# LANL-Seismoacoustics/GeoAc

Measured on AMD Instinct MI355X. Metric: RK4 ray-steps/sec, GeoAcGlobal 360x90 ToyAtmo fan; arrivals within 1e-6 of ref, higher is better.
Workload: dtype f64; 1 GPU; GeoAcGlobal -prop ToyAtmo.met, 360 az x 90 incl = 32400 rays (phi step 1 deg), bounces=2, CalcAmp=True, WriteRays=False, rng_max=1500; rays_per_gpu=32400, ray_steps_per_pass=874273730, parallelism=azimuth-sharded x1

## Files before the change

geoac_amd/csrc/geoac_api.cpp:

```cpp
#include <hip/hip_runtime.h>
#include <math.h>
#include <cmath>
#include <stdio.h>
#include <stdlib.h>
#include <string.h>
#include <ctype.h>
#include <errno.h>
#include <algorithm>
#include <atomic>
#include <memory>
#include <mutex>
#include <string>
#include <thread>
#include <vector>

#include "../../include/geoac_hip.h"
#include "../../include/geoac_probe.h"
#include "../../include/geoac_host.h"
#include "geoac_device.h"
#include "geoac_map_int.h"
#include "geoac_stations_int.h"
#include "geoac_tubemap_int.h"
#include "geoac_refine_int.h"

// ... 120 lines not shown
    hipStream_t pp_stream = nullptr;
    hipStream_t acc_stream = nullptr;
    std::vector<hipEvent_t> evp;
    hipStream_t rk4b_stream = nullptr;
    std::vector<hipEvent_t> evj;
    DevBuf ev_row[3], ev_m[3], ev_amp[3], nev[3], smp_out;
    long long smp_cap = 4ll << 20;
    unsigned long long n_samples = 0;
    unsigned long long* h_counters = nullptr;
    int n_rays = 0, n_pad = 0, legs = 0;
    double ms_total = 0, ms_rk4 = 0, ms_post = 0;
    unsigned long long n_epochs = 0, path_bytes_w = 0, path_bytes_r = 0, total_steps = 0, err_flags = 0;
    int s_rows_override = 0;
    bool no_overlap = false;
    int pp_blocks = 0;
    double pair_frac = -1.0;
    double stagger_frac = -1.0;
    double stagger_rows = -1.0;
    double hybrid_rows = -1.0;
    bool two_chunks = false;
    bool trace_epochs = false;
    bool no_gate = false;
    bool no_pair = false;
    bool grid_build_host = false;
    int ev_slack = 72;
    int trio = 0;
    int duo = 0;
    bool abs_table = true;
    DevBuf atab;
    std::vector<double> atab_mkey;
    DevBuf ppfix;
    double atab_tol = 1e-10;
    int ppfix_cap = 1 << 20;
    unsigned long long atmo_version = 0, atab_version = ~0ull;
    double atab_key[7] = {0, 0, 0, 0, 0, 0, 0};
    int atab_entries = 0, atab_flagged = 0;
    double atab_worst = 0;
    unsigned long long pp_fixup_segments = 0;
    int n_members = 1;
    int mem_slots = 0;
    std::vector<double> ens_T, ens_rho, ens_sl;
    std::vector<double> mconsts;
    DevBuf d_mconsts;
    int n_src = 1;
    std::vector<double> sources;
    int layout_members = 1;
// ... 64 lines not shown
const char* geoac_last_error(geoac_ctx* ctx){ return ctx ? ctx->err.c_str() : ""; }

int geoac_default_params(int eqset, geoac_params* p){
    if(!p) return GEOAC_E_INVALID;
    memset(p, 0, sizeof(*p));
    p->ds_min = 0.001; p->ds_max = 0.5;
    if(eqset == GEOAC_EQ_GLOBAL || eqset == GEOAC_EQ_GLOBAL_RNGDEP){
        p->ray_limit = 10000.0;
        p->range_limit = 1500.0;
        p->r_earth = 6370.0;
        p->src[0] = 0.0; p->src[1] = 30.0; p->src[2] = 0.0;
    } else {
        p->ray_limit = 5000.0;
        p->range_limit = 10000.0;
        p->r_earth = 0.0;
    }
    p->vert_limit = NAN;
    p->z_grnd = 0.0; p->tweak_abs = 0.3; p->freq = 0.1;
    p->bounces = 2; p->calc_amp = 1; p->mode = 0; p->sample_stride = 25;
    for(int q = 0; q < 4; q++) p->xy_limits[q] = NAN;
    return GEOAC_OK;
}

static const char* const kOptionNames[] = {
    "S_ROWS", "NO_OVERLAP", "PP_BLOCKS", "ABS_TABLE", "ABS_TABLE_TOL", "PPFIX_CAP", "DUO", "TRIO", "EV_SLACK", "NO_PAIR", "PAIR_FRAC", "HYBRID_ROWS", "STAGGER_FRAC", "STAGGER_ROWS", "TWO_CHUNKS", "TRACE_EPOCHS", "NO_GATE", "SORT", "TILE", "PP_ONETRIP", "PP_LDS_TABLE", "PP_LDS_PAD", "CU_SPLIT", "CHUNK_GIB", "ACCUM_BATCH",
    "NO_QUAD", "GRID_LANES", "OCT", "HEX", "SPREAD", "COMPACT", "QUAD_CACHE", "GRID_COOP", "SUB_EPOCHS", "SUB_MIN_WAVES", "SUB_TEST_STALL", "SMP_CAP", "GRID_BUILD", nullptr };
const char* const* geoac_option_names(void){ return kOptionNames; }

int geoac_set_option(geoac_ctx* ctx, const char* key, const char* value){
    if(!ctx || !key || !value) return GEOAC_E_INVALID;
    std::string k(key);
    if(k.rfind("GEOAC_", 0) == 0) k = k.substr(6);
    for(char& c : k) c = (char)toupper((unsigned char)c);
    bool int_ok = false, dbl_ok = false;
    long long lv = 0; double dv = 0.0;
    { char* end = nullptr; errno = 0; lv = strtoll(value, &end, 10); int_ok = (end != value && *end == 0 && errno == 0); }
    { char* end = nullptr; errno = 0; dv = strtod(value, &end); dbl_ok = (end != value && *end == 0 && errno == 0 && dv == dv); }
    const int iv = (int)lv;
    auto bad = [&](const char* want){ return fail(ctx, GEOAC_E_INVALID, "set_option: " + k + "=" + value + ": expected " + want); };
    auto flag = [&](bool& dst) -> int { if(!int_ok || (lv != 0 && lv != 1)) return bad("0 or 1"); dst = lv != 0; return GEOAC_OK; };
    if(k == "S_ROWS"){ if(!int_ok || lv < 0 || lv > 0x7fffffff) return bad("a row count >= 0 (0: sized from the free memory)"); ctx->s_rows_override = iv; }
    else if(k == "NO_OVERLAP") return flag(ctx->no_overlap);
    else if(k == "PP_BLOCKS"){ if(!int_ok || lv < 0 || lv > 0x7fffffff) return bad("a block count >= 0"); ctx->pp_blocks = iv; }
    else if(k == "ABS_TABLE") return flag(ctx->abs_table);
    else if(k == "ABS_TABLE_TOL"){ if(!dbl_ok || !(dv > 0.0)) return bad("a tolerance > 0"); ctx->atab_tol = dv; }
    else if(k == "PPFIX_CAP"){ if(!int_ok || lv <= 0 || lv > 0x3fffffff) return bad("a capacity > 0"); ctx->ppfix_cap = iv; }
    else if(k == "DUO"){
        if(!int_ok || lv < 0 || lv > 3) return bad("0..3");
        if(lv && !geoac_build_has_ab()) return fail(ctx, GEOAC_E_UNSUPPORTED, "set_option: DUO: the wave-specialised kernel is part of A/B builds only (make AB=1)");
        ctx->duo = iv;
    }
    else if(k == "TRIO"){
        if(!int_ok || lv < 0 || lv > 31) return bad("0, 1 (3, 5, 11, 27: timing diagnostics)");
        if(lv && !geoac_build_has_ab()) return fail(ctx, GEOAC_E_UNSUPPORTED, "set_option: TRIO: the three-wave kernel is part of A/B builds only (make AB=1)");
        ctx->trio = iv;
    }
    else if(k == "EV_SLACK"){ if(!int_ok || lv < 0 || lv > 1000000) return bad("a slot count >= 0"); ctx->ev_slack = iv; }
    else if(k == "NO_PAIR") return flag(ctx->no_pair);
    else if(k == "PAIR_FRAC"){ if(!dbl_ok || dv < 0.0 || dv > 1.0) return bad("a share in [0, 1]"); ctx->pair_frac = dv; }
    else if(k == "STAGGER_FRAC"){ if(!dbl_ok || dv < -1.0 || dv > 0.9) return bad("a share in [0, 0.9] (0: off), or -1 (by launch plan)"); ctx->stagger_frac = dv; }
    else if(k == "STAGGER_ROWS"){ if(!dbl_ok || !(dv > 0.0 && dv <= 1.0)) return bad("a ratio in (0, 1]"); ctx->stagger_rows = dv; }
    else if(k == "HYBRID_ROWS"){ if(!dbl_ok || !(dv > 0.0 && dv <= 1.0)) return bad("a ratio in (0, 1]"); ctx->hybrid_rows = dv; }
    else if(k == "TWO_CHUNKS") return flag(ctx->two_chunks);
    else if(k == "TRACE_EPOCHS") return flag(ctx->trace_epochs);
    else if(k == "NO_GATE") return flag(ctx->no_gate);
    else if(k == "SORT") return flag(ctx->sort_rays);
    else if(k == "TILE") return flag(ctx->tile_rays);
    else if(k == "PP_ONETRIP"){ if(!int_ok || lv < -1 || lv > 1) return bad("0, 1 or -1 (by launch plan)"); ctx->pp_onetrip = iv; }
    else if(k == "CHUNK_GIB"){ if(!int_ok || lv < 1 || lv > 256) return bad("GiB per path chunk in 1 .. 256"); ctx->chunk_gib = iv; }
    else if(k == "ACCUM_BATCH"){ if(!int_ok || lv < -1 || lv > 1) return bad("0, 1 or -1 (by launch plan: the late epochs)"); ctx->accum_batch = iv; }
    else if(k == "CU_SPLIT"){ if(!int_ok || lv < -1 || lv > 248) return bad("compute units for the post-pass, 0 .. 248 (0: no partition), or -1 (by launch plan)"); ctx->cu_split = iv; }
    else if(k == "PP_LDS_PAD"){ if(!int_ok || lv < -1 || lv > 160 * 1024) return bad("bytes of LDS in 0 .. 163840, or -1 (by launch plan)"); ctx->pp_lds_pad = iv; }
    else if(k == "PP_LDS_TABLE"){ if(!int_ok || lv < -1 || lv > 1) return bad("0, 1 or -1 (by launch plan)"); ctx->pp_lds_table = iv; }
    else if(k == "NO_QUAD") return flag(ctx->no_quad);
    else if(k == "GRID_LANES"){
        if(!int_ok || !(iv == 0 || iv == 1 || iv == 2 || iv == 4 || iv == 8 || iv == 16)) return bad("0, 1, 2, 4, 8 or 16");
        if(iv == 2 && !geoac_build_has_ab()) return fail(ctx, GEOAC_E_UNSUPPORTED, "set_option: GRID_LANES=2: the grid sets' two-lane kernels are part of A/B builds only (make AB=1)");
        ctx->grid_lanes = iv;
    }
    else if(k == "OCT") return flag(ctx->oct);
    else if(k == "HEX") return flag(ctx->hex);
    else if(k == "SPREAD"){ if(!int_ok || lv < 0 || lv > 64 || (lv & (lv - 1))) return bad("0 (by launch plan) or a power of two up to 64"); ctx->spread_override = iv; }
    else if(k == "COMPACT") return flag(ctx->compact);
    else if(k == "QUAD_CACHE") return flag(ctx->quad_cache);
    else if(k == "GRID_COOP") return flag(ctx->grid_coop);
    else if(k == "SUB_EPOCHS"){ if(!int_ok || lv < 1 || lv > 16) return bad("1..16"); ctx->sub_epochs = iv; }
// ... 472 lines not shown
    const bool is_global = (ctx->eqset == GEOAC_EQ_GLOBAL);
    const bool is_sph = is_global || ctx->eqset == GEOAC_EQ_GLOBAL_RNGDEP;
    if(is_global){ P.E = p.calc_amp ? 18 : 6; P.pathw = 6; }
    else if(ctx->eqset == GEOAC_EQ_3D){ P.E = p.calc_amp ? 12 : 4; P.pathw = 4; }
    else if(is_grid){ P.E = p.calc_amp ? 18 : 6; P.pathw = 6; }
    else { P.E = p.calc_amp ? 6 : 3; P.pathw = 2; }
    P.rays_form = ((p.mode & (GEOAC_MODE_WRITE_RAYS | GEOAC_MODE_WRITE_CAUSTICS)) != 0 || ctx->eqset == GEOAC_EQ_2D) ? 1 : 0;
    P.nseg = ctx->n_nodes - 1;
    P.step_limit = (long long)(p.ray_limit * (int)(1.0 / (p.ds_min * 10)));
    if(P.step_limit > 0x7fffffffLL) P.step_limit = 0x7fffffffLL;
    if(P.step_limit < 2) P.step_limit = 2;
    P.x_min = ctx->x[0]; P.x_max = ctx->x[ctx->n_nodes - 1];
    P.ds_min = p.ds_min; P.ds_max = p.ds_max;
    P.r_earth = is_sph ? p.r_earth : 0.0; P.z_grnd = p.z_grnd;
    P.ground = P.r_earth + p.z_grnd;
    P.vert_limit = p.vert_limit; P.range_limit = p.range_limit;
    if(p.range_limit >= 0.0){ const double l2 = p.range_limit * p.range_limit; P.range_sq[0] = l2 * (1.0 - 1e-12); P.range_sq[1] = l2 * (1.0 + 1e-12); }
    else { P.range_sq[0] = 0.0; P.range_sq[1] = -1.0; }
    if(is_global){
        double half = p.range_limit / (2.0 * p.r_earth);
        if(half >= kPi / 2.0){ P.range_thresh = 2.0; P.range_skip = 1e300; }
        else if(half <= 0.0){ P.range_thresh = -1.0; P.range_skip = -1.0; }
        else { double s = sin(half); P.range_thresh = s * s; P.range_skip = half * (1.0 - 1e-9); }
    }
    P.src[0] = p.src[0]; P.src[1] = p.src[1]; P.src[2] = p.src[2];
    P.freq = p.freq; P.tweak_abs = p.tweak_abs;
    {
        P.sb_const[0] = pow(10.0, -0.67887); P.sb_const[1] = pow(10.0, -0.10744); P.sb_const[2] = pow(10, -3.3979);
        P.sb_const[3] = 5.0 / sqrt(21.0); P.sb_const[4] = sqrt(3.0 / 7.0);
        P.src_trig[0] = sin(p.src[1] * kPi / 180.0); P.src_trig[1] = cos(p.src[1] * kPi / 180.0);
        if(is_grid){ P.T_o = P.P_o = 0.0; P.c000 = 0.0; } else {
        const size_t nn = (size_t)ctx->n_nodes;
        ctx->mconsts.assign((size_t)K * GEOAC_MEMP, 0.0);
        std::vector<double> Tm, rm;
        for(int m = 0; m < K; m++){
        const bool prof = K > 1;
        if(prof){ Tm.assign(ctx->ens_T.begin() + m * nn, ctx->ens_T.begin() + (m + 1) * nn); rm.assign(ctx->ens_rho.begin() + m * nn, ctx->ens_rho.begin() + (m + 1) * nn); }
        const std::vector<double>& Tv = prof ? Tm : ctx->T;
        const std::vector<double>& rv = prof ? rm : ctx->rho;
        const double* slm = prof ? ctx->ens_sl.data() + 4 * nn * m : ctx->sl.data();
        double Tg = host_spline_f(ctx->x, Tv, slm, p.z_grnd);
        double rg = host_spline_f(ctx->x, rv, slm + 3 * nn, p.z_grnd);
        double cg = sqrt(kGamR * Tg) * 1000.0;
        P.T_o = cg * cg / (kRgas * kGam);
        P.cbrt_To = cbrt(P.T_o);
        P.P_o = rg * (cg * cg) / kGam * 1000.0;
// ... 744 lines not shown
```

geoac_amd/csrc/geoac_device.h:

```cpp
#ifndef GEOAC_DEVICE_H_
#define GEOAC_DEVICE_H_

#include <stdint.h>

#define GEOAC_SEGW      14
#define GEOAC_MAXE      18
#define GEOAC_MAXLEGS   64
#define GEOAC_ATABW     20
#define GEOAC_LAT_OFF   1024
#define GEOAC_LAT_N     2049
#define GEOAC_PP_ROWS   16
#define GEOAC_CNT_PPFLAG 28

enum {
    ST_Y0     = 0,
    ST_K      = 18,
    ST_LEG    = 19,
    ST_DONE   = 20,
    ST_HMAX   = 21,
    ST_C0     = 22,
    ST_NU0    = 23,
    ST_AUX0   = 24,
    ST_SEG    = 30,
    ST_TT     = 31,
    ST_AT     = 32,
    ST_PLEG   = 33,
    ST_LTT    = 34,
    ST_LAT    = 35,
    ST_YM2    = 36,
    ST_DPREV  = 54,
    ST_NSTATE = 55
};

struct GeoacDevParams {
// ... 2 lines not shown
    int     E, pathw;
    int     nseg;
    int     s_rows;
    int     table_in_lds;
    int     live_slot;
    int     slot_lo, slot_hi;
    int     lanes_per_ray;
    int     duo;
    int     trio;
    int     spread;
    int     quad_cache;
    int     coop;
    int     seg_safe;
    int     pp_blocks;
    int     rays_form;
    long long step_limit;
    double  x_min, x_max;
    double  ds_min, ds_max;
    double  ground;
    double  r_earth, z_grnd;
    double  vert_limit, range_limit, range_thresh;
    double  range_sq[2];
    double  range_skip;
    double  src[3];
    double  freq, tweak_abs;
    double  T_o, P_o;
    double  cbrt_To;
    double  c000;
    double  src_trig[2];
    double  sb_const[5];
    const double* seg;
    const double* rho;
    int*    ppfix;
    int     ppfix_cap;
    int     pp_lds_pad;
    int     accum_batch;
    int     pp_lds_table;
    int     pp_onetrip;
    const double* atab;
    const double* lat_trig;
    int           atab_on;
    double        atab_D;
    double        atab_lo;
    double        seg_per_x;
    int           gnx, gny;
    double        g_lo[2], g_hi[2];
// ... 55 lines not shown
```

geoac_amd/csrc/geoac_kernels.hip:

```cpp
#include <hip/hip_runtime.h>
#include <math.h>
#include <type_traits>
#include "geoac_device.h"
#include "../../include/geoac_hip.h"

#define DEVINL __device__ __forceinline__
#ifndef GEOAC_CACHE_REG_STATE
#define GEOAC_CACHE_REG_STATE 0
#endif
#ifndef GEOAC_OCT_LDS_STATE
#define GEOAC_OCT_LDS_STATE 0
#endif
#define GEOAC_ROT_MAX 1.0e-3

#pragma clang fp contract(off)

#ifndef GEOAC_RCPC
#define GEOAC_RCPC 1
#endif
#ifndef GEOAC_RCPC_EMAX
#define GEOAC_RCPC_EMAX 1.0e-5
#endif
#ifndef GEOAC_AB
#define GEOAC_AB 0
#endif

static constexpr double kPi   = 3.141592653589793238462643;
static constexpr double kGam  = 1.4;
static constexpr double kRgas = 287.05;
static constexpr double kGamR = 0.00040187;

DEVINL double frcp(double x){
    double r = __builtin_amdgcn_rcp(x);
    double e = __builtin_fma(-x, r, 1.0);
    double t = __builtin_fma(e, e, e);
    return __builtin_fma(r, t, r);
}
DEVINL double frsq(double x){
    double y = __builtin_amdgcn_rsq(x);
    double g = x * y;
    double e = __builtin_fma(-g, y, 1.0);
    double p = __builtin_fma(e, 0.375, 0.5);
    return __builtin_fma(y * e, p, y);
}
// ... 185 lines not shown
    double t = x - s[0];
    return __builtin_fma(t, __builtin_fma(t, __builtin_fma(t, q[3], q[2]), q[1]), q[0]);
}

DEVINL void member_view(GeoacDevParams& P, int m){
    const int k = m % P.n_profiles;
    P.seg += (size_t)k * P.nseg * GEOAC_SEGW;
    P.rho += (size_t)k * P.nseg * 4;
    if(P.atab) P.atab += (size_t)k * (P.nseg + 2) * GEOAC_ATABW;
    const double* c = P.mem_consts + (size_t)m * GEOAC_MEMC;
    P.T_o = c[0]; P.P_o = c[1]; P.cbrt_To = c[2]; P.c000 = c[3];
    P.src[0] = c[4]; P.src[1] = c[5]; P.src[2] = c[6];
    P.src_trig[0] = c[7]; P.src_trig[1] = c[8];
}
DEVINL int member_of_slot(const GeoacDevParams& P, int slot){
    const int m = __builtin_amdgcn_readfirstlane(slot) / P.mem_slots;
    return m < P.n_members ? m : P.n_members - 1;
}

struct GlobalStage { double n0, n1, n2, inm, cn, icg, dc, du, dv, v, cg2, ir, ico, sth, cth, H0, K2; };
#define GEOAC_GSTAGE_W 17

struct NoHook { DEVINL void operator()() const {} };
template <bool AMP, int W, typename TabPtr, class HOOK = NoHook, bool ROT0 = false, bool LOCATED = false>
DEVINL void global_base(TabPtr tab, const GeoacDevParams& P, int& seg, double* rec, const double* y, double sth0, double cth0, double dlat, double* dy, GlobalStage& S, const HOOK& hook = HOOK(), double* rcp0 = nullptr, bool first = false){
    const double r = y[0];
    const double n0 = y[3], n1 = y[4], n2 = y[5];
    const double xe = clampq(r, P.x_min, P.x_max);
    double sth, cth;
    if(ROT0){ sth = sth0; cth = cth0; }
    else rot_small(sth0, cth0, dlat, sth, cth);
    const double nn  = __builtin_fma(n0, n0, __builtin_fma(n1, n1, n2 * n2));
    const double inm0 = frsq(nn);
#if GEOAC_RCPC
    double ir, ico;
    if(ROT0 || first){ ir = frcp(r); ico = frcp(cth); rcp0[0] = ir; rcp0[1] = ico; }
    else {
        const double e1 = __builtin_fma(-r, rcp0[0], 1.0), e2 = __builtin_fma(-cth, rcp0[1], 1.0);
        ir = __builtin_fma(rcp0[0], __builtin_fma(e1, e1, e1), rcp0[0]);
        ico = __builtin_fma(rcp0[1], __builtin_fma(e2, e2, e2), rcp0[1]);
        if(__builtin_expect(!(fabs(e2) <= GEOAC_RCPC_EMAX), 0)) ico = frcp(cth);
    }
#else
    const double ir  = frcp(r);
    const double ico = frcp(cth);
#endif
    Atm9 a;
    if(LOCATED) seg_eval_at(rec, xe, a); else seg_cached_eval<W>(tab, P, xe, seg, rec, a);
    hook();
    const double inm = inm0, numag = nn * inm;
    const double u = a.u, v = a.v, du = a.du, dv = a.dv;

    const double qT  = kGamR * a.T;
    const double ic  = frsq(qT);
    const double c   = qT * ic;
    const double hc  = (0.5 * kGamR) * ic;
    const double dc  = hc * a.dT;
    const double cn  = c * inm;
    const double cg0 = cn * n0;
    const double cg1 = __builtin_fma(cn, n1, v);
    const double cg2 = __builtin_fma(cn, n2, u);
    const double icg = frsq(__builtin_fma(cg0, cg0, __builtin_fma(cg1, cg1, cg2 * cg2)));
    const double tn  = sth * ico;
    const double u0 = cg0 * icg, u1 = cg1 * icg, u2 = cg2 * icg;
// ... 52 lines not shown
    const double dcg2 = __builtin_fma(R0, du, a2);
    const double e   = icg * __builtin_fma(D.u0, dcg0, __builtin_fma(D.u1, dcg1, D.u2 * dcg2));
    const double w0 = __builtin_fma(icg, dcg0, -D.u0 * e);
    const double w1 = __builtin_fma(icg, dcg1, -D.u1 * e);
    const double w2 = __builtin_fma(icg, dcg2, -D.u2 * e);
    const double dG1 = -R0 * D.ir2;
    const double dG2 = D.G2 * __builtin_fma(D.tn, R1, -R0 * ir);
    const double s22 = __builtin_fma(m2, cg2, n2 * dcg2);
    const double dT0 = __builtin_fma(dG1, D.nc12, ir * __builtin_fma(m1, D.cg1, __builtin_fma(n1, dcg1, s22)));
    const double dT1 = __builtin_fma(-D.cnn1, m0, __builtin_fma(-n0, a1, __builtin_fma(D.tn, s22, (D.n2cg2 * R1) * D.ico2)));
    const double dncs = __builtin_fma(m0, cth, __builtin_fma(m1, sth, R1 * __builtin_fma(n1, cth, -n0 * sth)));
    const double dT2 = -__builtin_fma(__builtin_fma(m2, v, n2 * dva), sth,
                         __builtin_fma((n2 * v) * R1, cth, __builtin_fma(a2, D.ncs, D.cnn2 * dncs)));

    dya[0] = w0;
    dya[1] = __builtin_fma(dG1, D.u1, G1 * w1);
    dya[2] = __builtin_fma(dG2, D.u2, D.G2 * w2);
    dya[3] = icg * (__builtin_fma(e, H0, -dT0)
                    - __builtin_fma(dnu, dc, __builtin_fma(m1, dv, __builtin_fma(m2, du, R0 * K2))));
    dya[4] = -icg * __builtin_fma(dG1, D.T1, G1 * dT1);
    dya[5] = -icg * __builtin_fma(dG2, D.T2, D.G2 * dT2);
}

template <bool AMP, int NQ, bool ROT0 = false, typename TabPtr>
DEVINL void global_rhs(TabPtr tab, const GeoacDevParams& P, int& seg, double* rec, const double* y, double sth0, double cth0, double dlat, double* dy, double* rcp0 = nullptr){
    GlobalStage S;
    global_base<AMP, GEOAC_SEGW, TabPtr, NoHook, ROT0>(tab, P, seg, rec, y, sth0, cth0, dlat, dy, S, NoHook(), rcp0);
    if(AMP){
        GlobalDerived D;
        global_derive(S, D);
        #pragma unroll
        for(int q = 0; q < NQ; q++) global_aux(S, D, y + 6 + 6 * q, dy + 6 + 6 * q);
    }
}

struct Medium { double c, dc, u, du, v, dv, rho; };
DEVINL Medium medium_at(const GeoacDevParams& P, double x){
    double xe = clampd(x, P.x_min, P.x_max);
    int k = seg_guess(P.seg, P, xe);
    Atm9 a; seg_eval<false>(P.seg, k, xe, a);
    Medium m;
    m.c = sqrt(kGamR * a.T); m.dc = kGamR / (2.0 * m.c) * a.dT;
    m.u = a.u; m.du = a.du; m.v = a.v; m.dv = a.dv;
    m.rho = rho_eval(P, k, xe);
    return m;
}

DEVINL double global_jacobian(const Medium& m, const double* y){
    double r = y[0], th = y[1];
    double nu_mag = sqrt(y[3] * y[3] + y[4] * y[4] + y[5] * y[5]);
// ... 278 lines not shown
        double MS = 1.0 + (nu0[0] * Mach[0] + nu0[1] * Mach[1] + nu0[2] * Mach[2]);
        y[0] = r0; y[1] = lat0; y[2] = lon0;
        for(int e = 0; e < 3; e++) y[3 + e] = nu0[e] / MS;
        if(AMP){
            double dlt = mlt[0] * Mach[0] + mlt[1] * Mach[1] + mlt[2] * Mach[2];
            double dlp = mlp[0] * Mach[0] + mlp[1] * Mach[1] + mlp[2] * Mach[2];
            for(int e = 0; e < 3; e++){
                y[9 + e]  = mlt[e] / MS - nu0[e] / (MS * MS) * dlt;
                y[15 + e] = mlp[e] / MS - nu0[e] / (MS * MS) * dlp;
            }
        }
        C.c0 = c0; C.nu0 = 1.0 / MS;
        C.a[0] = lat0; fsincos(lat0, C.a[1], C.a[2]);
        C.a[3] = 0.0; C.a[4] = 0.0; C.a[5] = 1.0;
        resume(P, C, y);
    }
    static DEVINL void fan_init(const GeoacDevParams& P){}
    static DEVINL double height(const GeoacDevParams& P, const double* y){ return y[0] - P.r_earth; }
    static DEVINL double above_ground(const GeoacDevParams& P, const double* y){ return y[0] - P.ground; }

    static DEVINL void resume(const GeoacDevParams& P, RayCtx& C, const double* y){
        rot_small(C.a[1], C.a[2], y[1] - C.a[0], C.cur[0], C.cur[1]);
    }
    template <typename TabPtr>
    static DEVINL void rhs(TabPtr tab, const GeoacDevParams& P, int& seg, const RayCtx& C, const double* y0, const double* yt, int stage, double* dy){
        if(stage == 0) global_rhs<AMP, 2, true>(tab, P, seg, C.rec, yt, C.cur[0], C.cur[1], 0.0, dy, C.rcp0);
        else global_rhs<AMP, 2>(tab, P, seg, C.rec, yt, C.cur[0], C.cur[1], yt[1] - y0[1], dy, C.rcp0);
    }
    static DEVINL void checks(const GeoacDevParams& P, RayCtx& C, const double* y, const double* yn, int k, bool& brk, bool& gnd){
        const double lon0 = P.src[2] * kPi / 180.0;
        const double dl = yn[1] - C.a[0], pl = yn[2] - lon0;
        if(__builtin_expect(fabs(dl) > GEOAC_ROT_MAX, 0)){ C.a[0] = yn[1]; fsincos(yn[1], C.a[1], C.a[2]); C.t[0] = C.a[1]; C.t[1] = C.a[2]; }
        else rot_small(C.a[1], C.a[2], dl, C.t[0], C.t[1]);
        bool far = false;
        if(fabs(yn[1] - P.src[1] * kPi / 180.0) * 0.5 + fabs(pl) * 0.5 >= P.range_skip){
            const double dp = pl - C.a[3];
            double tp0, tp1;
            if(__builtin_expect(fabs(dp) > GEOAC_ROT_MAX, 0)){ C.a[3] = pl; fsincos(pl, C.a[4], C.a[5]); tp0 = C.a[4]; tp1 = C.a[5]; }
            else rot_small(C.a[4], C.a[5], dp, tp0, tp1);
            const double sl0 = P.src_trig[0], cl0 = P.src_trig[1];
            double hav = __builtin_fma(cl0 * C.t[1], 0.5 * (1.0 - tp1), 0.5 * (1.0 - __builtin_fma(C.t[1], cl0, C.t[0] * sl0)));
            far = hav > P.range_thresh;
        }
        brk = (yn[0] > P.vert_limit) || far;
        gnd = yn[0] < P.ground;
    }
    static DEVINL void accept(RayCtx& C){ C.cur[0] = C.t[0]; C.cur[1] = C.t[1]; }
    static DEVINL void restart(const GeoacDevParams& P, RayCtx& C, const double* y){
        C.a[0] = y[1]; fsincos(y[1], C.a[1], C.a[2]);
        C.a[3] = y[2] - P.src[2] * kPi / 180.0; fsincos(C.a[3], C.a[4], C.a[5]);
        C.cur[0] = C.a[1]; C.cur[1] = C.a[2];
    }
    static DEVINL void arrival(const GeoacDevParams& P, const RayCtx& C, int slot, const double* yn, double* R){
        const double lat0 = P.src[1] * kPi / 180.0, lon0 = P.src[2] * kPi / 180.0;
        Medium m = medium_at(P, yn[0]);
        double z_src = P.src[0] < P.z_grnd ? P.z_grnd : P.src[0];
        double incl = -asin(m.c / C.c0 * yn[3]) * 180.0 / kPi;
        double baz = 90.0 - atan2(-yn[4], -yn[5]) * 180.0 / kPi;
        if(baz < -180.0) baz += 360.0;
        if(baz > 180.0) baz -= 360.0;
        double g1 = sin((yn[1] - lat0) / 2.0); g1 *= g1;
        double g2 = sin((yn[2] - lon0) / 2.0); g2 = cos(lat0) * cos(yn[1]) * g2 * g2;
        R[GEOAC_REC_INCL] = incl;
        R[GEOAC_REC_BACKAZ] = baz;
        R[GEOAC_REC_RANGE] = 2.0 * P.r_earth * asin(sqrt(g1 + g2));
        if(AMP){
            double amp, D;
            amp_jac(P, C, slot, yn, amp, D);
            R[GEOAC_REC_AMP] = amp;
// ... 52 lines not shown
        G.a0 = an0 + (B[3] - an0) / 2.0; G.a1 = an1 + (B[4] - an1) / 2.0; G.a2 = an2 + (B[5] - an2) / 2.0;
        G.a3 = frsq(G.a0 * G.a0 + G.a1 * G.a1 + G.a2 * G.a2);
        G.x = r;
    }
    static DEVINL double pp_tt(const GeoacDevParams& P, const double* aux, const PPGeom& G, double T, double u, double v){
        double qT = kGamR * T;
        double cn = (qT * frsq(qT)) * G.a3;
        double cp0 = cn * G.a0, cp1 = cn * G.a1 + v, cp2 = cn * G.a2 + u;
        return G.ds_tt * frsq(cp0 * cp0 + cp1 * cp1 + cp2 * cp2);
    }
    static DEVINL void segment(const GeoacDevParams& P, const double* st, size_t np, const double* a, const double* b, double& tt, double& at){
        double A[6], B[6];
        #pragma unroll
        for(int c = 0; c < 6; c++){ A[c] = a[c * np]; B[c] = b[c * np]; }
        pp_exact<EqGlobal<AMP_>>(P, nullptr, A, B, tt, at);
    }
};


struct EqGlobalPair : EqGlobal<true> {
    using Full = EqGlobal<true>;
    static constexpr int E = 12, LANES = 2;
    static constexpr bool SPLIT = true; static constexpr bool ROW_SPLIT = true;
    template <typename TabPtr>
    static DEVINL void rhs(TabPtr tab, const GeoacDevParams& P, int& seg, const RayCtx& C, const double* y0, const double* yt, int stage, double* dy){
        if(stage == 0) global_rhs<true, 1, true>(tab, P, seg, C.rec, yt, C.cur[0], C.cur[1], 0.0, dy, C.rcp0);
        else global_rhs<true, 1>(tab, P, seg, C.rec, yt, C.cur[0], C.cur[1], yt[1] - y0[1], dy, C.rcp0);
    }
    static DEVINL void reflect(const GeoacDevParams& P, const RayCtx& C, const double* yn, double* y, const double* ym2){
        double dr_k = yn[0] - y[0];
        double dr_g = y[0] - P.ground;
        double prev[E];
        #pragma unroll
        for(int e = 0; e < E; e++) prev[e] = y[e] + (y[e] - yn[e]) / dr_k * dr_g;
        Medium mr = medium_at(P, prev[0]);
        double c_ref = mr.c;
        double dnu_r_ds = -1.0 / c_ref * (C.c0 / c_ref * mr.dc + prev[4] * mr.dv + prev[5] * mr.du
                                          + c_ref / prev[0] * (prev[4] * prev[4] + prev[5] * prev[5]));
        #pragma unroll
        for(int e = 0; e < E; e++) y[e] = prev[e];
        y[0] = P.ground;
        y[3] = -prev[3];
        y[6] = -prev[6];
        y[9] = -prev[9] + 2.0 * dnu_r_ds * prev[6] / (c_ref / C.c0 * prev[3]);
    }
};

#pragma clang fp contract(fast)
#include "geoac_rngdep.h"
#ifndef GEOAC_CELL_REGS
// ... 408 lines not shown
        C.a[0] = nu0[0] / M; C.a[1] = nu0[1] / M;
        C.a[2] = mth[0] / M - nu0[0] / (M * M) * dMt;  C.a[3] = mth[1] / M - nu0[1] / (M * M) * dMt;
        C.a[4] = mph[0] / M - nu0[0] / (M * M) * dMp;  C.a[5] = mph[1] / M - nu0[1] / (M * M) * dMp;
        y[0] = P.src[0]; y[1] = P.src[1]; y[2] = z0; y[3] = nu0[2] / M;
        if(AMP){
            y[7]  = mth[2] / M - nu0[2] / (M * M) * dMt;
            y[11] = mph[2] / M - nu0[2] / (M * M) * dMp;
        }
    }
    static DEVINL void fan_init(const GeoacDevParams& P){}
    static DEVINL double height(const GeoacDevParams& P, const double* y){ return y[2]; }
    static DEVINL double above_ground(const GeoacDevParams& P, const double* y){ return y[2] - P.ground; }
    template <typename TabPtr>
    static DEVINL void rhs(TabPtr tab, const GeoacDevParams& P, int& seg, const RayCtx& C, const double* y0, const double* yt, int stage, double* dy){
        cart3_rhs<AMP>(tab, P, seg, C, yt, dy);
    }
    static DEVINL void checks(const GeoacDevParams& P, RayCtx& C, const double* y, const double* yn, int k, bool& brk, bool& gnd){
        const double s2 = yn[0] * yn[0] + yn[1] * yn[1];
        bool far = s2 > P.range_sq[1];
        if(__builtin_expect((s2 >= P.range_sq[0]) & (s2 <= P.range_sq[1]), 0)) far = sqrt(s2) > P.range_limit;
        brk = (yn[2] > P.vert_limit) || far;
        gnd = yn[2] < P.ground;
    }
    static DEVINL void accept(RayCtx& C){}
    static DEVINL void resume(const GeoacDevParams& P, RayCtx& C, const double* y){}
    static DEVINL void restart(const GeoacDevParams& P, RayCtx& C, const double* y){}
    static DEVINL void arrival(const GeoacDevParams& P, const RayCtx& C, int slot, const double* yn, double* R){
        double z0 = P.z_grnd < P.src[2] ? P.src[2] : P.z_grnd;
        Medium mg = medium_at(P, P.z_grnd);
        double incl = -asin(mg.c / C.c0 * yn[3]) * 180.0 / kPi;
        double baz = P.phi_deg[slot] + 180.0;
        while(baz > 180.0) baz -= 360.0;
        while(baz < -180.0) baz += 360.0;
        R[GEOAC_REC_INCL] = incl;
        R[GEOAC_REC_BACKAZ] = baz;
        R[GEOAC_REC_RANGE] = sqrt(yn[0] * yn[0] + yn[1] * yn[1]);
        if(AMP){
            double amp, D;
            amp_jac(P, C, slot, yn, amp, D);
            R[GEOAC_REC_AMP] = amp;
            R[GEOAC_REC_JACOB] = D;
        }
    }
    static DEVINL void amp_jac(const GeoacDevParams& P, const RayCtx& C, int slot, const double* yn, double& amp, double& D){
        double z0 = P.z_grnd < P.src[2] ? P.src[2] : P.z_grnd;
        Medium m = medium_at(P, yn[2]);
// ... 95 lines not shown
    static constexpr bool SPLIT = false;
    static constexpr bool KM2 = true, KM2_MEM = false, HMAX_PER_LEG = false;

    static DEVINL void init(const GeoacDevParams& P, double th, double ph, double* y, RayCtx& C){
        double z0 = P.src[0] < P.z_grnd ? P.z_grnd : P.src[0];
        Medium m = medium_at(P, z0);
        C.a[0] = cos(ph); C.a[1] = sin(ph); C.a[2] = cos(th); C.a[3] = sin(th); C.a[4] = 0.0; C.a[5] = 0.0;
        C.c0 = m.c + m.u * C.a[0] + m.v * C.a[1];
        C.nu0 = 1.0 / C.c0;
        y[0] = 0.0; y[1] = z0; y[2] = C.a[3];
        if(AMP) y[5] = C.a[2];
    }
    static DEVINL void fan_init(const GeoacDevParams& P){}
    static DEVINL double height(const GeoacDevParams& P, const double* y){ return y[1]; }
    static DEVINL double above_ground(const GeoacDevParams& P, const double* y){ return y[1] - P.ground; }
    template <typename TabPtr>
    static DEVINL void rhs(TabPtr tab, const GeoacDevParams& P, int& seg, const RayCtx& C, const double* y0, const double* yt, int stage, double* dy){
        cart2_rhs<AMP>(tab, P, seg, C, yt, dy);
    }
    static DEVINL void checks(const GeoacDevParams& P, RayCtx& C, const double* y, const double* yn, int k, bool& brk, bool& gnd){
        brk = (yn[1] > P.vert_limit) || (yn[0] > P.range_limit);
        gnd = yn[1] < P.ground;
    }
    static DEVINL void accept(RayCtx& C){}
    static DEVINL void resume(const GeoacDevParams& P, RayCtx& C, const double* y){}
    static DEVINL void restart(const GeoacDevParams& P, RayCtx& C, const double* y){}
    static DEVINL void arrival(const GeoacDevParams& P, const RayCtx& C, int slot, const double* yn, double* R){
        R[GEOAC_REC_INCL] = -P.theta_deg[slot];
        R[GEOAC_REC_BACKAZ] = 0.0;
        R[GEOAC_REC_RANGE] = yn[0];
        if(AMP){
            double amp, D;
            amp_jac(P, C, slot, yn, amp, D);
            R[GEOAC_REC_AMP] = amp;
            R[GEOAC_REC_JACOB] = D;
        }
    }
    static DEVINL void amp_jac(const GeoacDevParams& P, const RayCtx& C, int slot, const double* yn, double& amp, double& D){
        Medium m = medium_at(P, yn[1]);
        Medium mg = medium_at(P, P.z_grnd);
        double drds = m.c / C.c0 * C.a[2];
        double dzds = m.c / C.c0 * yn[2];
        D = yn[0] * (drds * yn[4] - dzds * yn[3]);
        double num = m.rho * m.c * C.a[2];
        double den = mg.rho * C.c0 * D;
        amp = 1.0 / (4.0 * kPi) * sqrt(fabs(num / den));
// ... 270 lines not shown
            R[GEOAC_REC_VALID] = 1.0;
            if(lim && !gnd){
                const double hl = EQ::height(P, yb);
                if(!(EQ::PW == 2 && (P.mode & GEOAC_MODE_INTERACTIVE))) hmax = (hmax < hl) ? hl : hmax;
            }
            R[GEOAC_REC_TURN] = hmax;
            if(leg >= P.bounces){
                done = true;
            } else {
                if(EQ::KM2 && EQ::KM2_MEM){
                    double r2[E];
                    #pragma unroll
                    for(int e = 0; e < E; e++) r2[e] = st[(ST_YM2 + ((EQ::SPLIT && e >= EQ::NB) ? e + EQ::NS * qs : e)) * np];
                    EQ::reflect(P, C, yb, ya, r2);
                } else EQ::reflect(P, C, yb, ya, yc);
                leg++; k = 0;
                EQ::restart(P, C, ya);
                put_row(ya);
            }
        }
    };

    if constexpr (EQ::SEG1D){
        while(__any((nr + 2 <= P.s_rows) && !done)){
            bool ev = false, pend = false;
            double dy[E], ys[E], w6 = 0.0;
            if((nr + 2 <= P.s_rows) && !done) for(;;){
                open_step(y);
                const double ds = set_ds(EQ::above_ground(P, y), P.ds_min, P.ds_max);
                const double ds_2 = 0.5 * ds, ds_6 = (1.0 / 6.0) * ds, ds_3 = (1.0 / 3.0) * ds;
                double yt[E];
                if(LDS) EQ::rhs(lds_tab, P, seg, C, y, y, 0, dy); else EQ::rhs(gtab, P, seg, C, y, y, 0, dy);
                #pragma unroll
                for(int e = 0; e < E; e++){ ys[e] = __builtin_fma(dy[e], ds_6, y[e]); yt[e] = __builtin_fma(dy[e], ds_2, y[e]); }
                #pragma unroll 1
                for(int stage = 1; stage < 3; stage++){
                    if(LDS) EQ::rhs(lds_tab, P, seg, C, y, yt, stage, dy); else EQ::rhs(gtab, P, seg, C, y, yt, stage, dy);
                    const double wa = (stage == 2) ? ds : ds_2;
                    #pragma unroll
                    for(int e = 0; e < E; e++){ ys[e] = __builtin_fma(dy[e], ds_3, ys[e]); yt[e] = __builtin_fma(dy[e], wa, y[e]); }
                }
                if(LDS) EQ::rhs(lds_tab, P, seg, C, y, yt, 3, dy); else EQ::rhs(gtab, P, seg, C, y, yt, 3, dy);
                double t[EQ::NB];
                #pragma unroll
                for(int e = 0; e < EQ::NB; e++) t[e] = __builtin_fma(dy[e], ds_6, ys[e]);
                EQ::checks(P, C, y, t, k + 1, brk, gnd);
                lim = (k + 1 >= k_lim);
                ev = brk || gnd || lim;
                const bool full = !(nr + 3 <= P.s_rows);
                if(__builtin_expect(__any(ev || full), 0)){ pend = true; w6 = ds_6; break; }
                #pragma unroll
                for(int e = 0; e < E; e++){
                    if(YM2_REG) ym2[e] = y[e];
                    y[e] = __builtin_fma(dy[e], ds_6, ys[e]);
                }
                k++; steps_here++;
                put_row(y);
                EQ::accept(C);
            }
            if(pend){
                #pragma unroll
                for(int e = 0; e < E; e++) ys[e] = __builtin_fma(dy[e], w6, ys[e]);
                k++; steps_here++;
                put_row(ys);
                EQ::accept(C);
                if(ev) leg_end(y, ys, ym2);
                else {
                    #pragma unroll
                    for(int e = 0; e < E; e++){ if(YM2_REG) ym2[e] = y[e]; y[e] = ys[e]; }
                }
            }
        }
    } else {
    double yn[E];
    while(EQ::COOP ? (bool)__any((nr + 2 <= row_end) && !done) : ((nr + 2 <= P.s_rows) && !done)){
        const bool act = EQ::COOP ? ((nr + 2 <= row_end) && !done) : true;
#ifdef GEOAC_KSTAT
        C.ckey = (C.ckey & ~1) | (act ? 1 : 0);
#endif
        double ds = P.ds_min;
        if(!EQ::COOP || act){
            open_step(y);
            ds = 0.05 - 0.049 * exp(-EQ::above_ground(P, y) / 0.75);
            ds = (P.ds_max < ds) ? P.ds_max : ds;
            ds = (ds < P.ds_min) ? P.ds_min : ds;
        }

        double dy[E], yt[E];
        #pragma unroll
        for(int e = 0; e < E; e++){ yt[e] = y[e]; yn[e] = y[e]; }
        if(EQ::LDS_STATE){
            #pragma unroll
            for(int e = 0; e < E; e++){ ly[e * 64] = y[e]; lyn[e * 64] = y[e]; }
        }
// ... 1254 lines not shown
```

include/geoac_probe.h:

```cpp
#ifndef GEOAC_PROBE_H_
#define GEOAC_PROBE_H_

#include "geoac_hip.h"

#ifdef __cplusplus
extern "C" {
#endif

int geoac_probe_atmo_1d(geoac_ctx* ctx, int n, const double* x, double* out9, double* rho);

int geoac_probe_absorption(geoac_ctx* ctx, int n, const double* x, const double* freq, double* alpha);

int geoac_probe_absorption_table(geoac_ctx* ctx, int n, const double* x, double* alpha);

int geoac_probe_grid(geoac_ctx* ctx, int n, const double* a0, const double* a1, const double* a2, int coop, double* out30, double* api7);

#ifdef __cplusplus
}
#endif
#endif
```

Measured before the change: 7.363 billion RK4 ray-steps/s.

## Add cheap range-check prefilter and drop reciprocal guard away from poles

Per-step range checks in the global 1D-segment stepping loop are replaced by a cheap planar distance test. The exact haversine range test now runs only when a ray nears the range limit, and such steps leave the fast loop. The guarded reciprocal fallback for cos(theta) is dropped from the RHS whenever no lane in the wave is near a pole, using a conservative pole bound computed on the host. Both are meant to cut per-step ALU work and branching in the RK4 inner loop. The cost is extra wave-wide votes, more exits from the fast loop, and added code size and register pressure from the template variants.

```diff
diff --git a/geoac_amd/csrc/geoac_api.cpp b/geoac_amd/csrc/geoac_api.cpp
--- a/geoac_amd/csrc/geoac_api.cpp
+++ b/geoac_amd/csrc/geoac_api.cpp
@@ -166,6 +166,8 @@
     bool trace_epochs = false;
     bool no_gate = false;
     bool no_pair = false;
+    bool range_skip = true;
+    bool pole_fast = true;
     bool grid_build_host = false;
     int ev_slack = 72;
     int trio = 0;
@@ -276,9 +278,32 @@
     return GEOAC_OK;
 }
 
+extern "C" void geoac_probe_step_vote_consts(double range_limit, double r_earth, double ground_radius, double ds_min, double ds_max, double* out){
+    const double half = range_limit / (2.0 * r_earth);
+    double thresh, skip2;
+    if(half >= kPi / 2.0){ thresh = 2.0; skip2 = 1e300; }
+    else if(half <= 0.0){ thresh = -1.0; skip2 = -1.0; }
+    else {
+        const double s = sin(half);
+        thresh = s * s;
+        skip2 = 4.0 * thresh * (1.0 - 1e-9) - 1e-14;
+        if(!(skip2 > 0.0)) skip2 = -1.0;
+    }
+    double pole_k = (double)INFINITY, delta = (double)INFINITY;
+    const double ds_top = ds_max < GEOAC_DS_TOP ? ds_max : GEOAC_DS_TOP;
+    const double dsb = ds_top > ds_min ? ds_top : ds_min;
+    const double r_lo = ground_radius - 2.0 * dsb;
+    if(dsb > 0.0 && r_lo - dsb > 0.0){
+        delta = dsb / (r_lo - dsb) * (1.0 + 1e-12);
+        const double t_max = (GEOAC_RCPC_EMAX - 0.5 * delta * delta - 1e-15) / delta;
+        if(t_max > 0.0) pole_k = (1.0 + 1e-12) / t_max;
+    }
+    out[0] = thresh; out[1] = skip2; out[2] = pole_k; out[3] = GEOAC_RCPC_EMAX; out[4] = delta;
+}
+
 static const char* const kOptionNames[] = {
     "S_ROWS", "NO_OVERLAP", "PP_BLOCKS", "ABS_TABLE", "ABS_TABLE_TOL", "PPFIX_CAP", "DUO", "TRIO", "EV_SLACK", "NO_PAIR", "PAIR_FRAC", "HYBRID_ROWS", "STAGGER_FRAC", "STAGGER_ROWS", "TWO_CHUNKS", "TRACE_EPOCHS", "NO_GATE", "SORT", "TILE", "PP_ONETRIP", "PP_LDS_TABLE", "PP_LDS_PAD", "CU_SPLIT", "CHUNK_GIB", "ACCUM_BATCH",
-    "NO_QUAD", "GRID_LANES", "OCT", "HEX", "SPREAD", "COMPACT", "QUAD_CACHE", "GRID_COOP", "SUB_EPOCHS", "SUB_MIN_WAVES", "SUB_TEST_STALL", "SMP_CAP", "GRID_BUILD", nullptr };
+    "NO_QUAD", "GRID_LANES", "OCT", "HEX", "SPREAD", "COMPACT", "QUAD_CACHE", "GRID_COOP", "SUB_EPOCHS", "SUB_MIN_WAVES", "SUB_TEST_STALL", "SMP_CAP", "GRID_BUILD", "RANGE_SKIP", "POLE_FAST", nullptr };
 const char* const* geoac_option_names(void){ return kOptionNames; }
 
 int geoac_set_option(geoac_ctx* ctx, const char* key, const char* value){
@@ -316,6 +341,8 @@
     else if(k == "STAGGER_ROWS"){ if(!dbl_ok || !(dv > 0.0 && dv <= 1.0)) return bad("a ratio in (0, 1]"); ctx->stagger_rows = dv; }
     else if(k == "HYBRID_ROWS"){ if(!dbl_ok || !(dv > 0.0 && dv <= 1.0)) return bad("a ratio in (0, 1]"); ctx->hybrid_rows = dv; }
     else if(k == "TWO_CHUNKS") return flag(ctx->two_chunks);
+    else if(k == "RANGE_SKIP") return flag(ctx->range_skip);
+    else if(k == "POLE_FAST") return flag(ctx->pole_fast);
     else if(k == "TRACE_EPOCHS") return flag(ctx->trace_epochs);
     else if(k == "NO_GATE") return flag(ctx->no_gate);
     else if(k == "SORT") return flag(ctx->sort_rays);
@@ -834,6 +861,10 @@
         if(half >= kPi / 2.0){ P.range_thresh = 2.0; P.range_skip = 1e300; }
         else if(half <= 0.0){ P.range_thresh = -1.0; P.range_skip = -1.0; }
         else { double s = sin(half); P.range_thresh = s * s; P.range_skip = half * (1.0 - 1e-9); }
+        double c[5];
+        geoac_probe_step_vote_consts(p.range_limit, p.r_earth, P.ground, p.ds_min, p.ds_max, c);
+        P.range_skip2 = ctx->range_skip ? c[1] : -1.0;
+        P.pole_k = ctx->pole_fast ? c[2] : (double)INFINITY;
     }
     P.src[0] = p.src[0]; P.src[1] = p.src[1]; P.src[2] = p.src[2];
     P.freq = p.freq; P.tweak_abs = p.tweak_abs;
diff --git a/geoac_amd/csrc/geoac_device.h b/geoac_amd/csrc/geoac_device.h
--- a/geoac_amd/csrc/geoac_device.h
+++ b/geoac_amd/csrc/geoac_device.h
@@ -10,6 +10,10 @@
 #define GEOAC_LAT_OFF   1024
 #define GEOAC_LAT_N     2049
 #define GEOAC_PP_ROWS   16
+#define GEOAC_DS_TOP    0.05
+#ifndef GEOAC_RCPC_EMAX
+#define GEOAC_RCPC_EMAX 1.0e-5
+#endif
 #define GEOAC_CNT_PPFLAG 28
 
 enum {
@@ -58,6 +62,8 @@
     double  vert_limit, range_limit, range_thresh;
     double  range_sq[2];
     double  range_skip;
+    double  range_skip2;
+    double  pole_k;
     double  src[3];
     double  freq, tweak_abs;
     double  T_o, P_o;
diff --git a/geoac_amd/csrc/geoac_kernels.hip b/geoac_amd/csrc/geoac_kernels.hip
--- a/geoac_amd/csrc/geoac_kernels.hip
+++ b/geoac_amd/csrc/geoac_kernels.hip
@@ -17,9 +17,6 @@
 
 #ifndef GEOAC_RCPC
 #define GEOAC_RCPC 1
-#endif
-#ifndef GEOAC_RCPC_EMAX
-#define GEOAC_RCPC_EMAX 1.0e-5
 #endif
 #ifndef GEOAC_AB
 #define GEOAC_AB 0
@@ -251,7 +248,8 @@
 #define GEOAC_GSTAGE_W 17
 
 struct NoHook { DEVINL void operator()() const {} };
-template <bool AMP, int W, typename TabPtr, class HOOK = NoHook, bool ROT0 = false, bool LOCATED = false>
+template <bool B> struct BoolC { static constexpr bool value = B; };
+template <bool AMP, int W, typename TabPtr, class HOOK = NoHook, bool ROT0 = false, bool LOCATED = false, bool GUARD = true>
 DEVINL void global_base(TabPtr tab, const GeoacDevParams& P, int& seg, double* rec, const double* y, double sth0, double cth0, double dlat, double* dy, GlobalStage& S, const HOOK& hook = HOOK(), double* rcp0 = nullptr, bool first = false){
     const double r = y[0];
     const double n0 = y[3], n1 = y[4], n2 = y[5];
@@ -268,7 +266,7 @@
         const double e1 = __builtin_fma(-r, rcp0[0], 1.0), e2 = __builtin_fma(-cth, rcp0[1], 1.0);
         ir = __builtin_fma(rcp0[0], __builtin_fma(e1, e1, e1), rcp0[0]);
         ico = __builtin_fma(rcp0[1], __builtin_fma(e2, e2, e2), rcp0[1]);
-        if(__builtin_expect(!(fabs(e2) <= GEOAC_RCPC_EMAX), 0)) ico = frcp(cth);
+        if(GUARD){ if(__builtin_expect(!(fabs(e2) <= GEOAC_RCPC_EMAX), 0)) ico = frcp(cth); }
     }
 #else
     const double ir  = frcp(r);
@@ -367,10 +365,10 @@
     dya[5] = -icg * __builtin_fma(dG2, D.T2, D.G2 * dT2);
 }
 
-template <bool AMP, int NQ, bool ROT0 = false, typename TabPtr>
+template <bool AMP, int NQ, bool ROT0 = false, bool GUARD = true, typename TabPtr>
 DEVINL void global_rhs(TabPtr tab, const GeoacDevParams& P, int& seg, double* rec, const double* y, double sth0, double cth0, double dlat, double* dy, double* rcp0 = nullptr){
     GlobalStage S;
-    global_base<AMP, GEOAC_SEGW, TabPtr, NoHook, ROT0>(tab, P, seg, rec, y, sth0, cth0, dlat, dy, S, NoHook(), rcp0);
+    global_base<AMP, GEOAC_SEGW, TabPtr, NoHook, ROT0, false, GUARD>(tab, P, seg, rec, y, sth0, cth0, dlat, dy, S, NoHook(), rcp0);
     if(AMP){
         GlobalDerived D;
         global_derive(S, D);
@@ -695,10 +693,14 @@
     static DEVINL void resume(const GeoacDevParams& P, RayCtx& C, const double* y){
         rot_small(C.a[1], C.a[2], y[1] - C.a[0], C.cur[0], C.cur[1]);
     }
+    template <bool GUARD, typename TabPtr>
+    static DEVINL void rhs_g(TabPtr tab, const GeoacDevParams& P, int& seg, const RayCtx& C, const double* y0, const double* yt, int stage, double* dy){
+        if(stage == 0) global_rhs<AMP, 2, true, GUARD>(tab, P, seg, C.rec, yt, C.cur[0], C.cur[1], 0.0, dy, C.rcp0);
+        else global_rhs<AMP, 2, false, GUARD>(tab, P, seg, C.rec, yt, C.cur[0], C.cur[1], yt[1] - y0[1], dy, C.rcp0);
+    }
     template <typename TabPtr>
     static DEVINL void rhs(TabPtr tab, const GeoacDevParams& P, int& seg, const RayCtx& C, const double* y0, const double* yt, int stage, double* dy){
-        if(stage == 0) global_rhs<AMP, 2, true>(tab, P, seg, C.rec, yt, C.cur[0], C.cur[1], 0.0, dy, C.rcp0);
-        else global_rhs<AMP, 2>(tab, P, seg, C.rec, yt, C.cur[0], C.cur[1], yt[1] - y0[1], dy, C.rcp0);
+        rhs_g<true>(tab, P, seg, C, y0, yt, stage, dy);
     }
     static DEVINL void checks(const GeoacDevParams& P, RayCtx& C, const double* y, const double* yn, int k, bool& brk, bool& gnd){
         const double lon0 = P.src[2] * kPi / 180.0;
@@ -706,18 +708,33 @@
         if(__builtin_expect(fabs(dl) > GEOAC_ROT_MAX, 0)){ C.a[0] = yn[1]; fsincos(yn[1], C.a[1], C.a[2]); C.t[0] = C.a[1]; C.t[1] = C.a[2]; }
         else rot_small(C.a[1], C.a[2], dl, C.t[0], C.t[1]);
         bool far = false;
-        if(fabs(yn[1] - P.src[1] * kPi / 180.0) * 0.5 + fabs(pl) * 0.5 >= P.range_skip){
-            const double dp = pl - C.a[3];
-            double tp0, tp1;
-            if(__builtin_expect(fabs(dp) > GEOAC_ROT_MAX, 0)){ C.a[3] = pl; fsincos(pl, C.a[4], C.a[5]); tp0 = C.a[4]; tp1 = C.a[5]; }
-            else rot_small(C.a[4], C.a[5], dp, tp0, tp1);
-            const double sl0 = P.src_trig[0], cl0 = P.src_trig[1];
-            double hav = __builtin_fma(cl0 * C.t[1], 0.5 * (1.0 - tp1), 0.5 * (1.0 - __builtin_fma(C.t[1], cl0, C.t[0] * sl0)));
-            far = hav > P.range_thresh;
-        }
+        if(fabs(yn[1] - P.src[1] * kPi / 180.0) * 0.5 + fabs(pl) * 0.5 >= P.range_skip) far = range_far(P, C, pl);
         brk = (yn[0] > P.vert_limit) || far;
         gnd = yn[0] < P.ground;
     }
+    static DEVINL bool range_far(const GeoacDevParams& P, RayCtx& C, double pl){
+        const double dp = pl - C.a[3];
+        double tp0, tp1;
+        if(__builtin_expect(fabs(dp) > GEOAC_ROT_MAX, 0)){ C.a[3] = pl; fsincos(pl, C.a[4], C.a[5]); tp0 = C.a[4]; tp1 = C.a[5]; }
+        else rot_small(C.a[4], C.a[5], dp, tp0, tp1);
+        const double sl0 = P.src_trig[0], cl0 = P.src_trig[1];
+        double hav = __builtin_fma(cl0 * C.t[1], 0.5 * (1.0 - tp1), 0.5 * (1.0 - __builtin_fma(C.t[1], cl0, C.t[0] * sl0)));
+        return hav > P.range_thresh;
+    }
+    static constexpr bool POLE_FAST = true;
+    template <bool POLE>
+    static DEVINL void checks_fast(const GeoacDevParams& P, RayCtx& C, const double* y, const double* yn, int k, bool& brk, bool& gnd, bool& slow){
+        const double dl = yn[1] - C.a[0];
+        rot_small(C.a[1], C.a[2], dl, C.t[0], C.t[1]);
+        if(__builtin_expect(fabs(dl) > GEOAC_ROT_MAX, 0)){ C.a[0] = yn[1]; fsincos(yn[1], C.a[1], C.a[2]); C.t[0] = C.a[1]; C.t[1] = C.a[2]; }
+        const double A = yn[1] - P.src[1] * kPi / 180.0, B = yn[2] - P.src[2] * kPi / 180.0;
+        const double q = __builtin_fma(fabs(P.src_trig[1] * C.t[1]), B * B, A * A);
+        slow = !(q < P.range_skip2);
+        if(POLE) slow = slow || !(fabs(C.t[0]) * P.pole_k <= fabs(C.t[1]));
+        brk = yn[0] > P.vert_limit;
+        gnd = yn[0] < P.ground;
+    }
+    static DEVINL bool near_pole(const GeoacDevParams& P, const RayCtx& C){ return !(fabs(C.cur[0]) * P.pole_k <= fabs(C.cur[1])); }
     static DEVINL void accept(RayCtx& C){ C.cur[0] = C.t[0]; C.cur[1] = C.t[1]; }
     static DEVINL void restart(const GeoacDevParams& P, RayCtx& C, const double* y){
         C.a[0] = y[1]; fsincos(y[1], C.a[1], C.a[2]);
@@ -816,10 +833,14 @@
     using Full = EqGlobal<true>;
     static constexpr int E = 12, LANES = 2;
     static constexpr bool SPLIT = true; static constexpr bool ROW_SPLIT = true;
+    template <bool GUARD, typename TabPtr>
+    static DEVINL void rhs_g(TabPtr tab, const GeoacDevParams& P, int& seg, const RayCtx& C, const double* y0, const double* yt, int stage, double* dy){
+        if(stage == 0) global_rhs<true, 1, true, GUARD>(tab, P, seg, C.rec, yt, C.cur[0], C.cur[1], 0.0, dy, C.rcp0);
+        else global_rhs<true, 1, false, GUARD>(tab, P, seg, C.rec, yt, C.cur[0], C.cur[1], yt[1] - y0[1], dy, C.rcp0);
+    }
     template <typename TabPtr>
     static DEVINL void rhs(TabPtr tab, const GeoacDevParams& P, int& seg, const RayCtx& C, const double* y0, const double* yt, int stage, double* dy){
-        if(stage == 0) global_rhs<true, 1, true>(tab, P, seg, C.rec, yt, C.cur[0], C.cur[1], 0.0, dy, C.rcp0);
-        else global_rhs<true, 1>(tab, P, seg, C.rec, yt, C.cur[0], C.cur[1], yt[1] - y0[1], dy, C.rcp0);
+        rhs_g<true>(tab, P, seg, C, y0, yt, stage, dy);
     }
     static DEVINL void reflect(const GeoacDevParams& P, const RayCtx& C, const double* yn, double* y, const double* ym2){
         double dr_k = yn[0] - y[0];
@@ -1274,6 +1295,8 @@
         brk = (yn[2] > P.vert_limit) || far;
         gnd = yn[2] < P.ground;
     }
+    static constexpr bool POLE_FAST = false;
+    static DEVINL void checks_fast(const GeoacDevParams& P, RayCtx& C, const double* y, const double* yn, int k, bool& brk, bool& gnd, bool& slow){ checks(P, C, y, yn, k, brk, gnd); slow = false; }
     static DEVINL void accept(RayCtx& C){}
     static DEVINL void resume(const GeoacDevParams& P, RayCtx& C, const double* y){}
     static DEVINL void restart(const GeoacDevParams& P, RayCtx& C, const double* y){}
@@ -1415,6 +1438,8 @@
         brk = (yn[1] > P.vert_limit) || (yn[0] > P.range_limit);
         gnd = yn[1] < P.ground;
     }
+    static constexpr bool POLE_FAST = false;
+    static DEVINL void checks_fast(const GeoacDevParams& P, RayCtx& C, const double* y, const double* yn, int k, bool& brk, bool& gnd, bool& slow){ checks(P, C, y, yn, k, brk, gnd); slow = false; }
     static DEVINL void accept(RayCtx& C){}
     static DEVINL void resume(const GeoacDevParams& P, RayCtx& C, const double* y){}
     static DEVINL void restart(const GeoacDevParams& P, RayCtx& C, const double* y){}
@@ -1731,8 +1756,9 @@
     };
 
     if constexpr (EQ::SEG1D){
+        if constexpr (!EQ::POLE_FAST){
         while(__any((nr + 2 <= P.s_rows) && !done)){
-            bool ev = false, pend = false;
+            bool ev = false, pend = false, slow = false;
             double dy[E], ys[E], w6 = 0.0;
             if((nr + 2 <= P.s_rows) && !done) for(;;){
                 open_step(y);
@@ -1753,11 +1779,11 @@
                 double t[EQ::NB];
                 #pragma unroll
                 for(int e = 0; e < EQ::NB; e++) t[e] = __builtin_fma(dy[e], ds_6, ys[e]);
-                EQ::checks(P, C, y, t, k + 1, brk, gnd);
+                EQ::checks_fast(P, C, y, t, k + 1, brk, gnd, slow);
                 lim = (k + 1 >= k_lim);
                 ev = brk || gnd || lim;
                 const bool full = !(nr + 3 <= P.s_rows);
-                if(__builtin_expect(__any(ev || full), 0)){ pend = true; w6 = ds_6; break; }
+                if(__builtin_expect(__any(ev || full || slow), 0)){ pend = true; w6 = ds_6; break; }
                 #pragma unroll
                 for(int e = 0; e < E; e++){
                     if(YM2_REG) ym2[e] = y[e];
@@ -1779,6 +1805,75 @@
                     for(int e = 0; e < E; e++){ if(YM2_REG) ym2[e] = y[e]; y[e] = ys[e]; }
                 }
             }
+        }
+        } else {
+        constexpr bool PF = !SMP;
+        while(__any((nr + 2 <= P.s_rows) && !done)){
+            bool ev = false, pend = false, slow = false;
+            double dy[E], ys[E], w6 = 0.0;
+            auto step_parts = [&](auto guard) -> double {
+                constexpr bool G = decltype(guard)::value;
+                auto rhs = [&](const double* yi, int stage){
+                    if(LDS) EQ::template rhs_g<G>(lds_tab, P, seg, C, y, yi, stage, dy); else EQ::template rhs_g<G>(gtab, P, seg, C, y, yi, stage, dy);
+                };
+                open_step(y);
+                const double ds = set_ds(EQ::above_ground(P, y), P.ds_min, P.ds_max);
+                const double ds_2 = 0.5 * ds, ds_6 = (1.0 / 6.0) * ds, ds_3 = (1.0 / 3.0) * ds;
+                double yt[E];
+                rhs(y, 0);
+                #pragma unroll
+                for(int e = 0; e < E; e++){ ys[e] = __builtin_fma(dy[e], ds_6, y[e]); yt[e] = __builtin_fma(dy[e], ds_2, y[e]); }
+                #pragma unroll 1
+                for(int stage = 1; stage < 3; stage++){
+                    rhs(yt, stage);
+                    const double wa = (stage == 2) ? ds : ds_2;
+                    #pragma unroll
+                    for(int e = 0; e < E; e++){ ys[e] = __builtin_fma(dy[e], ds_3, ys[e]); yt[e] = __builtin_fma(dy[e], wa, y[e]); }
+                }
+                rhs(yt, 3);
+                double t[EQ::NB];
+                #pragma unroll
+                for(int e = 0; e < EQ::NB; e++) t[e] = __builtin_fma(dy[e], ds_6, ys[e]);
+                EQ::template checks_fast<PF>(P, C, y, t, k + 1, brk, gnd, slow);
+                lim = (k + 1 >= k_lim);
+                ev = brk || gnd || lim;
+                return ds_6;
+            };
+            const bool act = (nr + 2 <= P.s_rows) && !done;
+            bool guarded = false;
+            if constexpr (PF) guarded = __any(act && EQ::near_pole(P, C));
+            if(!guarded){
+                if(act) for(;;){
+                    const double ds_6 = step_parts(BoolC<!PF>());
+                    const bool full = !(nr + 3 <= P.s_rows);
+                    if(__builtin_expect(__any(ev || full || slow), 0)){ pend = true; w6 = ds_6; break; }
+                    #pragma unroll
+                    for(int e = 0; e < E; e++){
+                        if(YM2_REG) ym2[e] = y[e];
+                        y[e] = __builtin_fma(dy[e], ds_6, ys[e]);
+                    }
+                    k++; steps_here++;
+                    put_row(y);
+                    EQ::accept(C);
+                }
+            } else if constexpr (PF){ if(act){ w6 = step_parts(BoolC<true>()); pend = true; } }
+            if(pend){
+                #pragma unroll
+                for(int e = 0; e < E; e++) ys[e] = __builtin_fma(dy[e], w6, ys[e]);
+                if(slow){
+                    brk = EQ::range_far(P, C, ys[2] - P.src[2] * kPi / 180.0) || brk;
+                    ev = brk || gnd || lim;
+                }
+                k++; steps_here++;
+                put_row(ys);
+                EQ::accept(C);
+                if(ev) leg_end(y, ys, ym2);
+                else {
+                    #pragma unroll
+                    for(int e = 0; e < E; e++){ if(YM2_REG) ym2[e] = y[e]; y[e] = ys[e]; }
+                }
+            }
+        }
         }
     } else {
     double yn[E];
diff --git a/include/geoac_probe.h b/include/geoac_probe.h
--- a/include/geoac_probe.h
+++ b/include/geoac_probe.h
@@ -15,6 +15,8 @@
 
 int geoac_probe_grid(geoac_ctx* ctx, int n, const double* a0, const double* a1, const double* a2, int coop, double* out30, double* api7);
 
+void geoac_probe_step_vote_consts(double range_limit, double r_earth, double ground_radius, double ds_min, double ds_max, double* out);
+
 #ifdef __cplusplus
 }
 #endif
```

Result: faster. 7.492 billion RK4 ray-steps/s, median of 6 (+1.7%).
